# JohnLonginotto/uq

Hardware: AMD Instinct MI355X
Metric: FASTQ encode MB/s (150bp synthetic; bit-exact tables vs reference) (higher is better)
Workload: dtype u8

## Files before the change

uq_amd/csrc/pack.hip:

```cpp
#include "common.h"
#include "swar.h"
#include "lines.h"
#include "histo.h"

#ifdef PK_ROLE_CLOCK
__device__ unsigned long long pk_role_clock[16];
#define PK_CLOCK(k) do { const uint64_t now_ = __builtin_readcyclecounter(); ck_sum[(k) - 1] += now_ - ck_prev; ck_prev = now_; if ((k) == 1) ++ck_tiles; } while (0)
extern "C" int uq_pack_role_clock(unsigned long long* out16, int reset) {
    if (out16 && hipMemcpyFromSymbol(out16, HIP_SYMBOL(pk_role_clock), sizeof(pk_role_clock)) != hipSuccess) return 1;
    if (reset) {
        const unsigned long long zero[16] = {0};
        if (hipMemcpyToSymbol(HIP_SYMBOL(pk_role_clock), zero, sizeof(zero)) != hipSuccess) return 1;
    }
    return 0;
}
#else
#define PK_CLOCK(k) do { } while (0)
#endif

namespace {
constexpr int PK_THREADS = 256;

struct PackLut {
    int16_t dna_code[256];
    int16_t qual_code[256];
    int16_t n_qual[256];
};

struct PackGeom {
    uint32_t R;
    uint32_t Rs;
    uint32_t Cd, Cq;
    uint32_t G;
    uint32_t variable;
    uint32_t stage_bytes;
    uint32_t out_bytes;
    uint32_t magicG;
    uint32_t dna_max;
    uint32_t fill_d, fill_q;
    uint32_t P, magicP;
    uint32_t q_addlo, q_addhi;
    uint32_t n_char, n_code;
    uint32_t n_qchar;
    uint32_t h_shift, i2c_lo, i2c_hi, c2c_lo, c2c_hi;
};

__device__ __forceinline__ uint32_t acgt_codes(uint32_t w) { return ((w ^ (w >> 1)) >> 1) & 0x03030303u; }
__device__ __forceinline__ uint32_t acgt_chars(uint32_t codes) { return __builtin_amdgcn_perm(0u, 0x54474341u, codes); }
template <int B>
__device__ __forceinline__ uint32_t pack4(uint32_t x) {
    if (B == 8) return __builtin_amdgcn_perm(0u, x, 0x00010203u);
#ifndef PK_OLD_PACK4
    if (B <= 2) return __builtin_amdgcn_udot4(x, (1u << (3 * B)) | (1u << (2 * B + 8)) | (1u << (B + 16)) | (1u << 24), 0u, false);
    {
        const uint32_t hi = __builtin_amdgcn_udot4(x, (1u << B) | (1u << 8), 0u, false);
        return __builtin_amdgcn_udot4(x, (1u << (B + 16)) | (1u << 24), hi << (2 * B), false);
    }
#endif
    if (B == 2) return (x * 0x40100401u) >> 24;
    const uint32_t c0 = x & ((1u << B) - 1), c1 = (x >> 8) & ((1u << B) - 1), c2 = (x >> 16) & ((1u << B) - 1), c3 = x >> 24;
    return (((((c0 << B) | c1) << B) | c2) << B) | c3;
}

template <int B>
__device__ __forceinline__ uint32_t group_byte(uint32_t a0, uint32_t a1, int i) {
#ifndef PK_OLD_STORE
    if constexpr ((4 * B) % 8 == 0) return i < B / 2 ? a1 >> (8 * i) : a0 >> (8 * (i - B / 2));
    else
#endif
    return (uint32_t)((((uint64_t)a0 << (4 * B)) | a1) >> (8 * i));
}

template <bool CLEAR = false>
__device__ __noinline__ void store_tile_any(uint8_t* gdst, uint8_t* lsrc, uint32_t nb, uint32_t tid) {
    const uint32_t mis = (uint32_t)(uintptr_t)gdst;
    if ((mis & 15) == 0) {
        const uint32_t nv = nb >> 4;
        for (uint32_t i = tid; i < nv; i += 256) { ((uint4*)gdst)[i] = ((const uint4*)lsrc)[i]; if (CLEAR) ((uint4*)lsrc)[i] = make_uint4(0, 0, 0, 0); }
        for (uint32_t i = (nv << 4) + tid; i < nb; i += 256) { gdst[i] = lsrc[i]; if (CLEAR) lsrc[i] = 0; }
    } else if ((mis & 7) == 0) {
        const uint32_t nv = nb >> 3;
        for (uint32_t i = tid; i < nv; i += 256) { ((uint2*)gdst)[i] = ((const uint2*)lsrc)[i]; if (CLEAR) ((uint2*)lsrc)[i] = make_uint2(0, 0); }
        for (uint32_t i = (nv << 3) + tid; i < nb; i += 256) { gdst[i] = lsrc[i]; if (CLEAR) lsrc[i] = 0; }
    } else if ((mis & 3) == 0) {
        const uint32_t nv = nb >> 2;
        for (uint32_t i = tid; i < nv; i += 256) { ((uint32_t*)gdst)[i] = ((const uint32_t*)lsrc)[i]; if (CLEAR) ((uint32_t*)lsrc)[i] = 0; }
        for (uint32_t i = (nv << 2) + tid; i < nb; i += 256) { gdst[i] = lsrc[i]; if (CLEAR) lsrc[i] = 0; }
    } else {
        for (uint32_t i = tid; i < nb; i += 256) { gdst[i] = lsrc[i]; if (CLEAR) lsrc[i] = 0; }
    }
}
template <bool CLEAR = false>
__device__ __forceinline__ void store_tile(uint8_t* gdst, uint8_t* lsrc, uint32_t nb, uint32_t tid) {
    if ((((uint32_t)(uintptr_t)gdst) & 15u) == 0 && (nb & 15u) == 0) {
#pragma unroll 1
        for (uint32_t i = tid; i < (nb >> 4); i += 256) { ((uint4*)gdst)[i] = ((const uint4*)lsrc)[i]; if (CLEAR) ((uint4*)lsrc)[i] = make_uint4(0, 0, 0, 0); }
    } else store_tile_any<CLEAR>(gdst, lsrc, nb, tid);
}

struct alignas(16) QnLds {
    uint8_t line1[256 + 16];
    uint8_t inset[256];
    uint8_t seps[32];
    uint32_t vmin[UQ_QF_MAXC], vmax[UQ_QF_MAXC];
    uint32_t flags, on, plen, slen, nsep, l1len;
    uint32_t sepset;
    uint32_t seps_lo, seps_hi;
    uint32_t pow10[10];
};

__device__ __forceinline__ uint32_t eq_bytes(uint32_t w, uint32_t c4) {
    const uint32_t x = w ^ c4;
    return ~((((x & 0x7F7F7F7Fu) + 0x7F7F7F7Fu) | x)) & 0x80808080u;
}
__device__ __forceinline__ uint32_t nondigit_bytes(uint32_t w) {
    const uint32_t lo7 = w & 0x7F7F7F7Fu;
    return (~(lo7 + 0x50505050u) | (lo7 + 0x46464646u) | w) & 0x80808080u;
}
__device__ __forceinline__ uint32_t low_bytes(uint32_t n) { return n >= 4 ? 0xFFFFFFFFu : ~(0xFFFFFFFFu << (8 * n)); }

__device__ __forceinline__ void lds_window12(const uint8_t* base, int32_t o, uint32_t& w0, uint32_t& w1, uint32_t& w2) {
    const uint32_t* p = (const uint32_t*)(base + (o & ~3));
    const uint32_t a = p[0], b = p[1], c = p[2], d = p[3];
    const uint32_t sh = (uint32_t)o & 3u;
    w0 = __builtin_amdgcn_alignbyte(b, a, sh);
    w1 = __builtin_amdgcn_alignbyte(c, b, sh);
    w2 = __builtin_amdgcn_alignbyte(d, c, sh);
}

__device__ __forceinline__ void qname_tile(const uint8_t* stage, const uint32_t* meta, uint32_t q, QnLds* s, uint32_t* __restrict__ vals, uint64_t pitch,
                                           uint64_t row) {
    const uint32_t qs = meta[4 * q], ql = meta[4 * q + 1] - qs - 1;
    const uint32_t plen = s->plen, slen = s->slen, nsep = s->nsep, l1len = s->l1len;
    uint32_t f = 0;
    if (ql > 255) f = 2;
    else if (ql < plen + slen) f = 8;
    else {
        for (uint32_t j = 0; j < plen; j += 8) {
            uint32_t a0, a1;
            lds_window8(stage, (int32_t)(qs + j), a0, a1);
            const uint32_t l0 = *(const uint32_t*)(s->line1 + j), l1 = *(const uint32_t*)(s->line1 + j + 4);
            const uint32_t left = plen - j;
            if (((a0 ^ l0) & low_bytes(left)) | ((a1 ^ l1) & (left > 4 ? low_bytes(left - 4) : 0u))) f |= 32u;
        }
        for (uint32_t j = 0; j < slen; j += 8) {
            uint32_t a0, a1, l0, l1;
            lds_window8(stage, (int32_t)(qs + ql - slen + j), a0, a1);
            lds_window8(s->line1, (int32_t)(l1len - slen + j), l0, l1);
            const uint32_t left = slen - j;
            if (((a0 ^ l0) & low_bytes(left)) | ((a1 ^ l1) & (left > 4 ? low_bytes(left - 4) : 0u))) f |= 64u;
        }
        const uint32_t end = ql - slen;
        const uint32_t sepset = s->sepset;
        const uint32_t c0 = 0x01010101u * (sepset & 0xFFu), c1 = 0x01010101u * ((sepset >> 8) & 0xFFu), c2 = 0x01010101u * ((sepset >> 16) & 0xFFu),
                       c3 = 0x01010101u * (sepset >> 24);
        unsigned long long epos = 0, eseq = 0;
        uint32_t found = 0, differs = 0, bad = 0;
        for (uint32_t w = plen; w < ql; w += 8) {
            uint32_t a0, a1, l0, l1;
            lds_window8(stage, (int32_t)(qs + w), a0, a1);
            lds_window8(s->line1, (int32_t)w, l0, l1);
            const uint32_t inl = ql - w;
            differs |= ((a0 ^ l0) & low_bytes(inl)) | ((a1 ^ l1) & (inl > 4 ? low_bytes(inl - 4) : 0u));
            if (w >= end) continue;
            const uint32_t inm = end - w;
            const uint32_t v0 = low_bytes(inm), v1 = inm > 4 ? low_bytes(inm - 4) : 0u;
            const uint32_t sm0 = (eq_bytes(a0, c0) | eq_bytes(a0, c1) | eq_bytes(a0, c2) | eq_bytes(a0, c3)) & v0;
            const uint32_t sm1 = (eq_bytes(a1, c0) | eq_bytes(a1, c1) | eq_bytes(a1, c2) | eq_bytes(a1, c3)) & v1;
            bad |= (nondigit_bytes(a0) & ~sm0 & v0) | (nondigit_bytes(a1) & ~sm1 & v1);
            unsigned long long m = (unsigned long long)sm0 | ((unsigned long long)sm1 << 32);
            const unsigned long long bytes = (unsigned long long)a0 | ((unsigned long long)a1 << 32);
            while (m) {
                const uint32_t k = ((uint32_t)__ffsll((long long)m) - 1u) >> 3;
                m &= m - 1;
                if (found < 8) {
                    epos |= (unsigned long long)(w + k) << (8 * found);
                    eseq |= ((bytes >> (8 * k)) & 0xFFull) << (8 * found);
                }
                ++found;
            }
        }
        if (bad) f |= 16u;
        const unsigned long long want = (unsigned long long)s->seps_lo | ((unsigned long long)s->seps_hi << 32);
        if (found != nsep || eseq != want) f |= 1u;
        uint32_t start = plen;
        for (uint32_t c = 0; c <= nsep && c < UQ_QF_MAXC; ++c) {
            uint32_t stop = c == nsep ? end : (uint32_t)(epos >> (8 * c)) & 0xFFu;
            if (stop < start || stop > end) stop = start;
            const uint32_t nd = stop - start;
            uint32_t w0, w1, w2;
            lds_window12(stage, (int32_t)(qs + stop) - 12, w0, w1, w2);
            const uint32_t keep = nd > 9 ? 9u : nd;
            const uint32_t k2 = low_bytes(keep >= 4 ? 0u : 4u - keep), k1 = keep <= 4 ? 0xFFFFFFFFu : (keep >= 8 ? 0u : low_bytes(8u - keep)),
                           k0 = keep <= 8 ? 0xFFFFFFFFu : low_bytes(12u - keep);
            const uint32_t d0 = w0 & 0x0F0F0F0Fu & ~k0, d1 = w1 & 0x0F0F0F0Fu & ~k1, d2 = w2 & 0x0F0F0F0Fu & ~k2;
            uint32_t mag = d0 >> 24;
            mag = mag * 10 + (d1 & 0xFFu); mag = mag * 10 + ((d1 >> 8) & 0xFFu); mag = mag * 10 + ((d1 >> 16) & 0xFFu); mag = mag * 10 + (d1 >> 24);
            mag = mag * 10 + (d2 & 0xFFu); mag = mag * 10 + ((d2 >> 8) & 0xFFu); mag = mag * 10 + ((d2 >> 16) & 0xFFu); mag = mag * 10 + (d2 >> 24);
            if (nd > 9) f |= 4u;
            else if (nd == 0 || (nd > 1 && mag < s->pow10[nd - 1])) f |= 16u;
            vals[c * pitch + row] = mag;
            if (mag < s->vmin[c]) atomicMin(&s->vmin[c], mag);
            if (mag > s->vmax[c]) atomicMax(&s->vmax[c], mag);
            start = stop + 1;
        }
        if (ql < l1len && !differs && !(f & 32u)) f |= 128u;
        if (ql < l1len && s->line1[l1len - ql] == s->line1[0]) f |= 128u;
    }
    if (f) atomicOr(&s->flags, f);
}

constexpr int PK_NV = 5;
constexpr int PK_NV_STATS = 4;
constexpr uint32_t pk_stage_bytes(bool stats) { return (uint32_t)(stats ? PK_NV_STATS : PK_NV) * PK_THREADS * 16 + 32; }
#ifdef PK_ONE_COPY
constexpr int pks_copies(int bd, bool four_wg) { return bd == 3 ? 4 : 1; }
#else
constexpr int pks_copies(int bd, bool four_wg) { return bd == 2 && four_wg ? 8 : 4; }
#endif
constexpr uint32_t pks_bins(int bd) { return bd == 3 ? 512u : 256u; }
constexpr uint32_t pks_words(int bd, bool four_wg) { return pks_bins(bd) * pks_copies(bd, four_wg) + 128; }

struct TileRec { uint64_t start; uint32_t T, A, B, pad; };
struct PkParked { unsigned long long* bad; uq_stats* st; uq_qname_fused* qf; uint64_t first, nb, nl_total; uint32_t Rs, pad; };
struct PackLists {
    CensusView cv;
    const uint32_t* over;
};

__global__ __launch_bounds__(256) void tile_origin_kernel(CensusView cv, const unsigned long long* __restrict__ d_async, const uint32_t* __restrict__ over, uint64_t first,
                                                          uint64_t n, uint64_t R, uint64_t entries, TileRec* __restrict__ rec, unsigned long long* __restrict__ bad) {
    const uint64_t tt = (uint64_t)blockIdx.x * 256 + threadIdx.x;
    if (tt == 0) *bad = UQ_NONE;
    if (tt >= entries) return;
    uint64_t nlines = 4 * (first + n);
    if (d_async) {
        nlines = d_async[0];
        const uint64_t have = nlines / 4;
        if (have < n) n = have;
        if (d_async[1] || *over) n = 0;
    }
    uint64_t r = tt * R;
    if (r > n) r = n;
    uint32_t T, kk;
    cv_locate(cv, (int64_t)(4 * (first + r)) - 1, T, kk);
    bool ok;
    TileRec out;
    out.start = n ? cv_line_start(cv, nlines, T, kk, 0, ok) : 0;
    uint32_t c[3];
#pragma unroll
    for (uint32_t k = 0; k < 3; ++k) {
        const uint64_t t = (uint64_t)T + k;
        c[k] = t < cv.nb ? (uint32_t)((t + 1 < cv.nb ? (uint64_t)cv.offs[t + 1] : nlines) - cv.offs[t]) : 0u;
        if (c[k] > CV_LIST_CAP) c[k] = CV_LIST_CAP;
    }
    out.T = T; out.A = kk | (c[0] << 16); out.B = c[1] | (c[2] << 16); out.pad = 0;
    rec[tt] = out;
}

template <int BD, int BQ, bool NTRICK, bool FAST, bool STATS, bool QN, bool LISTS = false, bool VAR = false>
__global__ __launch_bounds__(PK_THREADS, (STATS && (NTRICK || QN)) ? 4 : 5) void pack_tile_kernel(const uint8_t* __restrict__ buf,
                                                               const uint64_t* __restrict__ ls, uint64_t first,
                                                               uint64_t n, PackLut lut, PackGeom g,
                                                               uint8_t* __restrict__ dna, uint8_t* __restrict__ qual,
                                                               unsigned long long* __restrict__ bad,
                                                               uq_stats* __restrict__ st, const unsigned long long* __restrict__ d_async,
                                                               uq_qname_fused* __restrict__ qf, uint32_t* __restrict__ qvals, uint64_t qpitch, PackLists pl,
                                                               const TileRec* __restrict__ trec) {
    constexpr int NV = STATS ? PK_NV_STATS : PK_NV;
    extern __shared__ __align__(16) uint8_t smem[];
    constexpr uint32_t STAGE_BYTES = pk_stage_bytes(STATS);
    uint8_t* stage = smem + 16;
    int16_t* l_dna = (int16_t*)(stage + STAGE_BYTES);
    int16_t* l_qual = l_dna + 256;
    int16_t* l_nq = l_qual + 256;
    QnLds* qn = (QnLds*)(l_nq + 256);
    uint32_t* meta = (uint32_t*)((uint8_t*)qn + (STATS ? sizeof(QnLds) : 0));
    uint8_t* out_d = (uint8_t*)(meta + 4 * g.R + 4);

    const uint32_t tid = threadIdx.x;
    l_dna[tid] = lut.dna_code[tid];
    l_qual[tid] = lut.qual_code[tid];
    if (NTRICK) l_nq[tid] = lut.n_qual[tid];
    RecordAcc acc;
    bool incomplete = false;
    constexpr bool FOUR_WG = STATS && (NTRICK || QN);
    constexpr int PKS_COPIES = pks_copies(BD, FOUR_WG);
    __shared__ uint32_t cnt_tab[STATS ? pks_words(BD, FOUR_WG) : 1];
    uint32_t fill_pairs = 0, n_pairs = 0;
    constexpr uint32_t PKS_BINS = pks_bins(BD), PKS_WORDS = pks_words(BD, FOUR_WG);
    if (STATS) for (uint32_t i = tid; i < PKS_WORDS; i += PK_THREADS) cnt_tab[i] = 0;
    if (VAR) for (uint32_t i = tid; i < (g.out_bytes >> 4); i += PK_THREADS) ((uint4*)out_d)[i] = make_uint4(0, 0, 0, 0);
    bool qn_on = false;
    if (STATS && QN) qn_on = qf->ok != 0;
    if (STATS && QN) {
        qn->line1[tid] = qf->line1[tid]; qn->inset[tid] = qf->inset[tid];
        if (tid < 16) qn->line1[256 + tid] = 0;
        if (tid < 32) qn->seps[tid] = qf->seps[tid];
        if (tid < UQ_QF_MAXC) { qn->vmin[tid] = 0xFFFFFFFFu; qn->vmax[tid] = 0; }
        if (tid == 0) {
            qn->flags = 0; qn->plen = qf->plen; qn->slen = qf->slen; qn->nsep = qf->nsep; qn->l1len = qf->l1len;
            uint32_t set = 0x01010101u * qf->seps[0], nset = 1, lo = 0, hi = 0;
            for (uint32_t k = 0; k < qf->nsep && k < 8; ++k) {
                const uint32_t c = qf->seps[k];
                if (k < 4) lo |= c << (8 * k); else hi |= c << (8 * (k - 4));
                bool seen = false;
                for (uint32_t m = 0; m < nset; ++m) seen = seen || ((set >> (8 * m)) & 0xFFu) == c;
                if (!seen && nset < 4) { set = (set & ~(0xFFu << (8 * nset))) | (c << (8 * nset)); ++nset; }
            }
            qn->sepset = set; qn->seps_lo = lo; qn->seps_hi = hi;
            uint32_t pw = 1;
            for (uint32_t k = 0; k < 10; ++k) { qn->pow10[k] = pw; pw *= 10; }
        }
    }
    uint32_t nr = (uint32_t)n;
#if defined(__HIP_DEVICE_COMPILE__)
    asm("" : "+s"(nr));
#endif
    uint64_t nl_total = 4 * (first + n);
    constexpr bool lists = STATS && LISTS;
    if (d_async) {
        nl_total = d_async[0];
        const uint64_t have = d_async[0] / 4;
        if (have > nr) incomplete = true; else nr = (uint32_t)have;
        if (d_async[1] || (lists && *pl.over)) { incomplete = true; nr = 0; }
    }

    __shared__ PkParked parked;
    if constexpr (FOUR_WG) {
        if (tid == 0) { parked.bad = bad; parked.st = st; parked.qf = qf; parked.first = first; parked.nb = pl.cv.nb; parked.nl_total = nl_total; parked.Rs = g.Rs; }
    }
    auto p_bad = [&] { if constexpr (FOUR_WG) return parked.bad; else return bad; };
    auto p_st = [&] { if constexpr (FOUR_WG) return parked.st; else return st; };
    auto p_qf = [&] { if constexpr (FOUR_WG) return parked.qf; else return qf; };
    auto p_first = [&] { if constexpr (FOUR_WG) return parked.first; else return first; };
    auto p_nl_total = [&] { if constexpr (FOUR_WG) return parked.nl_total; else return nl_total; };
    auto p_Rs = [&] { if constexpr (FOUR_WG) return parked.Rs; else return g.Rs; };
    auto p_cv = [&] { CensusView v = pl.cv; if constexpr (FOUR_WG) v.nb = parked.nb; return v; };
    const uint32_t R = g.R;
    const uint32_t ntiles = (nr + R - 1) / R;
    const uint32_t S = gridDim.x;
    struct Bounds { uint64_t g0, g1; uint32_t pT, pA, pB; };
    struct Regs { uint4 v[NV]; uint64_t m0; uint64_t g0; uint32_t skew, nvec, Rt, mrel, mraw; bool ok; };
    struct RawBounds { uint32_t lo, hi; };
    auto load_raw = [&](uint32_t tt) {
        RawBounds x{0u, 0u};
        if (tt < ntiles) {
            const uint32_t ln = lane_id();
            if constexpr (lists) {
                x.lo = ((const uint32_t*)(trec + tt))[ln < 8u ? ln : 0u];
            } else {
                const uint32_t Rn = (nr - tt * R) < R ? (nr - tt * R) : R;
                const uint64_t v = ls[4 * (first + (uint64_t)tt * R) + (ln == 1u ? 4 * Rn : 0u)];
                x.lo = (uint32_t)v; x.hi = (uint32_t)(v >> 32);
            }
        }
        return x;
    };
    auto bounds_of = [&](uint32_t tt, const RawBounds& x) {
        auto lane = [](uint32_t v, int k) { return (uint32_t)__builtin_amdgcn_readlane((int)v, k); };
        Bounds b{0, 0, 0, 0, 0};
        if (tt < ntiles) {
            if constexpr (lists) {
                b.g0 = (uint64_t)lane(x.lo, 0) | ((uint64_t)lane(x.lo, 1) << 32);
                b.pT = lane(x.lo, 2); b.pA = lane(x.lo, 3); b.pB = lane(x.lo, 4);
                b.g1 = (uint64_t)lane(x.lo, 6) | ((uint64_t)lane(x.lo, 7) << 32);
            } else {
                b.g0 = (uint64_t)lane(x.lo, 0) | ((uint64_t)lane(x.hi, 0) << 32);
                b.g1 = (uint64_t)lane(x.lo, 1) | ((uint64_t)lane(x.hi, 1) << 32);
            }
        }
        return b;
    };
    auto load_bounds = [&](uint32_t tt) {
        Bounds b{0, 0, 0, 0, 0};
        if (tt < ntiles) {
            const uint32_t Rn = (nr - tt * R) < R ? (nr - tt * R) : R;
            if constexpr (lists) {
                const TileRec r0 = trec[tt];
                b.g0 = r0.start; b.pT = r0.T; b.pA = r0.A; b.pB = r0.B; b.g1 = trec[tt + 1].start;
            }
            else { b.g0 = ls[4 * (first + (uint64_t)tt * R)]; b.g1 = ls[4 * (first + (uint64_t)tt * R) + 4 * Rn]; }
        }
        return b;
    };
    auto tile_reads = [&](uint32_t tt) -> uint32_t { return tt < ntiles ? ((nr - tt * R) < R ? (nr - tt * R) : R) : 0u; };
    auto issue = [&](uint32_t rfirst, uint32_t cnt, Bounds b) {
        Regs x;
        x.ok = false; x.m0 = 0; x.g0 = b.g0; x.skew = 0; x.nvec = 0; x.Rt = 0; x.mrel = 0; x.mraw = 0;
#pragma unroll
        for (int u = 0; u < NV; ++u) x.v[u] = make_uint4(0, 0, 0, 0);
        if (cnt == 0) return x;
        x.Rt = cnt;
        const uint64_t a0 = ((uint64_t)(uintptr_t)buf + b.g0) & ~uint64_t(15);
        x.skew = (uint32_t)(((uint64_t)(uintptr_t)buf + b.g0) - a0);
        const uint64_t span = b.g1 - b.g0 + x.skew;
        x.nvec = (uint32_t)((span + 15) >> 4);
        x.ok = span + 32 <= STAGE_BYTES && x.nvec <= (uint32_t)(NV * PK_THREADS);
        if constexpr (lists) {
            const uint32_t kk = b.pA & 0xFFFFu, avail = (b.pA >> 16) + (b.pB & 0xFFFFu) + (b.pB >> 16);
            if (kk + 4 * cnt > avail) x.ok = false;
        }
        if (!x.ok) return x;
        const uint4* src = (const uint4*)(buf + ((int64_t)b.g0 - (int64_t)x.skew));
#pragma unroll
        for (int u = 0; u < NV; ++u) { const uint32_t i = u * PK_THREADS + tid; if (i < x.nvec) x.v[u] = src[i]; }
        if (tid <= 4 * x.Rt) {
            if constexpr (lists) {
                uint32_t idx = (b.pA & 0xFFFFu) + tid, t = b.pT;
                const uint32_t c0 = b.pA >> 16, c1 = b.pB & 0xFFFFu;
                if (idx > c0) { idx -= c0; ++t; if (idx > c1) { idx -= c1; ++t; } }
                x.mrel = x.skew - (uint32_t)b.g0 + (idx == 0 ? 0u : (uint32_t)t * (uint32_t)CV_TILE - pl.cv.mis + 1u);
                x.mraw = idx == 0 ? 0u : (uint32_t)pl.cv.list[(uint64_t)t * CV_LIST_CAP + (idx - 1)];
            } else x.m0 = ls[4 * (first + (uint64_t)rfirst) + tid];
        }
        return x;
    };

    uint32_t rr, pp;
    fast_divmod(tid, g.P, g.magicP, rr, pp);
    uint32_t badr = 0xFFFFFFFFu;
    uint32_t bad_tile = 0xFFFFFFFFu;
#ifdef PK_ROLE_CLOCK
    uint64_t ck_prev = 0, ck_sum[5] = {0, 0, 0, 0, 0};
    uint32_t ck_tiles = 0;
#endif
    auto do_tile = [&](const uint32_t r0, const Regs& cur, auto&& between) {
        const uint32_t Rt = cur.Rt;
        uint8_t* out_q = out_d + ((Rt * g.Cd + 15) & ~15u);
        if (cur.ok) {
            if (tid <= 4 * Rt) meta[tid] = lists ? cur.mrel + cur.mraw : (uint32_t)(cur.m0 - cur.g0) + cur.skew;
#pragma unroll
            for (int u = 0; u < NV; ++u) { const uint32_t i = u * PK_THREADS + tid; if (i < cur.nvec) ((uint4*)stage)[i] = cur.v[u]; }
        } else {
            if (tid == 0) bad_tile = bad_tile < r0 ? bad_tile : r0;
            incomplete = true;
            if (STATS && QN && qn_on && tid == 0) atomicOr(&p_qf()->flags, 256u);
        }
        __syncthreads();
        const bool ok = cur.ok;
        PK_CLOCK(1);
#ifndef PK_QN_NO_PRIO
        if (STATS && QN && tid >= PK_THREADS - 64) __builtin_amdgcn_s_setprio(3);
#endif
        between();
#ifndef PK_ABL_NOQN
        if (STATS && QN && qn_on && ok && tid >= PK_THREADS - 64 && tid - (PK_THREADS - 64) < Rt)
            qname_tile(stage, meta, tid - (PK_THREADS - 64), qn, qvals, qpitch, (uint64_t)r0 + (tid - (PK_THREADS - 64)));
#endif
#ifndef PK_QN_NO_PRIO
        if (STATS && QN && tid >= PK_THREADS - 64) __builtin_amdgcn_s_setprio(0);
#endif
        if (ok) {
            auto pack_group = [&](const uint32_t r, const uint32_t L, const int32_t wd, const uint32_t shd, const int32_t wq, const uint32_t shq, uint8_t* orow_d,
                                  uint8_t* orow_q, const uint32_t gg) {
                const int32_t j0 = (int32_t)L - 8 * (int32_t)gg - 8;
                uint32_t ad0 = 0, ad1 = 0, aq0 = 0, aq1 = 0;
                if (j0 > -8) {
                uint32_t b_lo, b_hi, q_lo, q_hi;
                lds_window8_at(stage, wd, shd, b_lo, b_hi);
                lds_window8_at(stage, wq, shq, q_lo, q_hi);
                if (j0 < 0) {
                    uint32_t mlo, mhi;
                    window_masks((uint32_t)(-j0), mlo, mhi);
                    b_lo = bfi(mlo, b_lo, g.fill_d); b_hi = bfi(mhi, b_hi, g.fill_d);
                    q_lo = bfi(mlo, q_lo, g.fill_q); q_hi = bfi(mhi, q_hi, g.fill_q);
                }
                bool generic = !FAST;
                if (FAST) {
                    uint32_t c0, c1, e0, e1;
                    if constexpr (BD == 2) {
                        c0 = acgt_codes(b_lo); c1 = acgt_codes(b_hi);
                        e0 = acgt_chars(c0) ^ b_lo; e1 = acgt_chars(c1) ^ b_hi;
                    } else {
                        c0 = __builtin_amdgcn_perm(g.i2c_hi, g.i2c_lo, (b_lo >> g.h_shift) & 0x07070707u);
                        c1 = __builtin_amdgcn_perm(g.i2c_hi, g.i2c_lo, (b_hi >> g.h_shift) & 0x07070707u);
                        e0 = __builtin_amdgcn_perm(g.c2c_hi, g.c2c_lo, c0) ^ b_lo; e1 = __builtin_amdgcn_perm(g.c2c_hi, g.c2c_lo, c1) ^ b_hi;
                    }
                    uint32_t u0 = q_lo + g.q_addlo, u1 = q_hi + g.q_addlo;
                    uint32_t bq0 = (q_lo | (q_lo + g.q_addhi) | ~u0) & 0x80808080u;
                    uint32_t bq1 = (q_hi | (q_hi + g.q_addhi) | ~u1) & 0x80808080u;
                    uint32_t x0 = u0 & 0x7F7F7F7Fu, x1 = u1 & 0x7F7F7F7Fu;
                    if (e0 | e1) {
                        if (NTRICK && !((q_lo | q_hi) & 0x80808080u)) {
                            const uint32_t m0 = nonzero_bytes(e0), m1 = nonzero_bytes(e1);
                            if (((b_lo ^ g.n_char) & m0) | ((b_hi ^ g.n_char) & m1)) generic = true;
                            c0 &= ~m0; c1 &= ~m1;
                            x0 = bfi(m0, g.n_code, x0); x1 = bfi(m1, g.n_code, x1);
                            bq0 &= ~m0; bq1 &= ~m1;
                        } else generic = true;
                    }
                    if (bq0 | bq1) generic = true;
                    ad0 = pack4<BD>(c0); ad1 = pack4<BD>(c1);
                    aq0 = pack4<BQ>(x0); aq1 = pack4<BQ>(x1);
                    if (STATS) {
                        if (generic) incomplete = true;
#ifdef PK_ABL_NOCOUNT
                        else if (false) {
#else
                        else {
#endif
                            uint8_t* hb = (uint8_t*)cnt_tab + ((lane_id() & (PKS_COPIES - 1)) << 2);
                            if constexpr (BD == 2) {
                                const uint32_t bin0 = (c0 << 6) | x0, bin1 = (c1 << 6) | x1;
#pragma unroll
                                for (int k = 0; k < 4; ++k) {
                                    if constexpr (PKS_COPIES == 1) {
                                        atomicAdd(&cnt_tab[(bin0 >> (8 * k)) & 0xFFu], 1u);
                                        atomicAdd(&cnt_tab[(bin1 >> (8 * k)) & 0xFFu], 1u);
                                    } else {
                                        atomicAdd((uint32_t*)(hb + (((bin0 >> (8 * k)) & 0xFFu) * (4 * PKS_COPIES))), 1u);
                                        atomicAdd((uint32_t*)(hb + (((bin1 >> (8 * k)) & 0xFFu) * (4 * PKS_COPIES))), 1u);
                                    }
                                }
                            } else {
#pragma unroll
                                for (int k = 0; k < 4; ++k) {
                                    const uint32_t b0 = (((c0 >> (8 * k)) & 7u) << 6) | ((x0 >> (8 * k)) & 63u), b1 = (((c1 >> (8 * k)) & 7u) << 6) | ((x1 >> (8 * k)) & 63u);
                                    atomicAdd((uint32_t*)(hb + b0 * (4 * PKS_COPIES)), 1u);
                                    atomicAdd((uint32_t*)(hb + b1 * (4 * PKS_COPIES)), 1u);
                                }
                            }
                            if (j0 < 0) fill_pairs += (uint32_t)(-j0);
                            if (NTRICK && (e0 | e1)) {
                                const uint32_t m0 = nonzero_bytes(e0), m1 = nonzero_bytes(e1);
                                const uint32_t ne0 = nonzero_bytes(q_lo ^ g.n_qchar), ne1 = nonzero_bytes(q_hi ^ g.n_qchar);
                                n_pairs += (uint32_t)__popc(m0 & 0x01010101u) + (uint32_t)__popc(m1 & 0x01010101u);
                                if ((m0 & ne0) | (m1 & ne1)) incomplete = true;
                            }
                        }
                    }
                }
                if (generic) {
                    const uint32_t cbw[2] = {b_lo, b_hi};
                    const uint32_t cqw[2] = {q_lo, q_hi};
                    uint32_t ad[2] = {0, 0}, aq[2] = {0, 0};
                    int32_t orall = 0;
#pragma unroll
                    for (int k = 0; k < 8; ++k) {
                        const uint32_t cb = (cbw[k >> 2] >> (8 * (k & 3))) & 255u;
                        const uint32_t cc = (cqw[k >> 2] >> (8 * (k & 3))) & 255u;
                        int32_t dc = l_dna[cb];
                        int32_t qc = l_qual[cc];
                        if (NTRICK) {
                            if (dc < 0) { dc = 0; qc = l_nq[cb]; }
                        }
                        orall |= dc | qc;
                        ad[k >> 2] = (ad[k >> 2] << BD) | (uint32_t)dc;
                        aq[k >> 2] = (aq[k >> 2] << BQ) | (uint32_t)qc;
                    }
                    if (orall < 0) {
                        badr = badr < r0 + r ? badr : r0 + r;
                        ad[0] = ad[1] = aq[0] = aq[1] = 0;
                    }
                    ad0 = ad[0]; ad1 = ad[1]; aq0 = aq[0]; aq1 = aq[1];
                }
                }
                if (g.variable) {
                    const int32_t i = (int32_t)L - 8 * (int32_t)gg;
                    if (i >= 0 && i < 4) { ad1 |= 1u << (BD * i); aq1 |= 1u << (BQ * i); }
                    else if (i >= 4 && i < 8) { ad0 |= 1u << (BD * (i - 4)); aq0 |= 1u << (BQ * (i - 4)); }
                }
                uint8_t* od = orow_d - BD * gg;
                uint8_t* oq = orow_q - BQ * gg;
#ifdef PK_ABL_NOSTORE
                if ((ad0 ^ aq0) == 0x12345678u && (ad1 ^ aq1) == 0x9ABCDEF0u) od[0] = 1;
                else if (false)
#endif
                if (gg + 1 < g.G) {
#pragma unroll
                    for (int i = 0; i < BD; ++i) od[-i] = (uint8_t)group_byte<BD>(ad0, ad1, i);
#pragma unroll
                    for (int i = 0; i < BQ; ++i) oq[-i] = (uint8_t)group_byte<BQ>(aq0, aq1, i);
                } else {
                    const uint32_t nd = g.Cd - BD * gg, nq = g.Cq - BQ * gg;
#pragma unroll
                    for (int i = 0; i < BD; ++i)
                        if ((uint32_t)i < nd) od[-i] = (uint8_t)group_byte<BD>(ad0, ad1, i);
#pragma unroll
                    for (int i = 0; i < BQ; ++i)
                        if ((uint32_t)i < nq) oq[-i] = (uint8_t)group_byte<BQ>(aq0, aq1, i);
                }
            };
            if (rr < Rt) {
                const uint32_t r = rr;
                const uint32_t so = meta[4 * r + 1];
                uint32_t L = meta[4 * r + 2] - so - 1;
                const uint32_t qo = meta[4 * r + 3];
                if (STATS) {
                    const uint32_t Lq = meta[4 * r + 4] - qo - 1;
#ifndef PK_ABL_NOREC
                    if (pp == 0) acc.record(r0 + r, stage[meta[4 * r + 2]] == '+', L, Lq, meta[4 * r + 4] - meta[4 * r]);
#endif
                    if (L > g.dna_max || Lq != L) incomplete = true;
                }
                if (L > g.dna_max || meta[4 * r + 4] - qo - 1 != L) { badr = badr < r0 + r ? badr : r0 + r; L = 0; }
                uint8_t* orow_d = out_d + r * g.Cd + (g.Cd - 1);
                uint8_t* orow_q = out_q + r * g.Cq + (g.Cq - 1);
                const uint32_t gend = VAR ? (((L + 8) >> 3) < g.G ? ((L + 8) >> 3) : g.G) : g.G;
#ifndef PK_ABL_NOGROUP
                int32_t wd = (int32_t)(so + L) - 8 * (int32_t)pp - 8, wq = (int32_t)(qo + L) - 8 * (int32_t)pp - 8;
                const uint32_t shd = (uint32_t)wd & 3u, shq = (uint32_t)wq & 3u;
                wd &= ~3; wq &= ~3;
                const int32_t wstep = 8 * (int32_t)g.P;
                for (uint32_t gg = pp; gg < gend; gg += g.P, wd -= wstep, wq -= wstep) pack_group(r, L, wd, shd, wq, shq, orow_d, orow_q, gg);
#endif
            }
        }
        PK_CLOCK(2);
        __syncthreads();
        PK_CLOCK(3);
#ifndef PK_NO_EARLY_WAIT
        __builtin_amdgcn_s_waitcnt(0x0F70);
#endif
        PK_CLOCK(4);
        if (ok) {
            if constexpr (STATS && (NTRICK || QN)) {
                store_tile<VAR>(dna + (uint64_t)r0 * g.Cd, out_d, Rt * g.Cd, tid);
                store_tile<VAR>(qual + (uint64_t)r0 * g.Cq, out_q, Rt * g.Cq, tid);
            } else {
                store_tile_any<VAR>(dna + (uint64_t)r0 * g.Cd, out_d, Rt * g.Cd, tid);
                store_tile_any<VAR>(qual + (uint64_t)r0 * g.Cq, out_q, Rt * g.Cq, tid);
            }
        }
        PK_CLOCK(5);
    };

    uint32_t t = blockIdx.x;
    constexpr bool VBOUNDS = STATS && (NTRICK || QN);
    using NextBounds = std::conditional_t<VBOUNDS, RawBounds, Bounds>;
    auto fetch_next = [&](uint32_t tt) -> NextBounds { if constexpr (VBOUNDS) return load_raw(tt); else return load_bounds(tt); };
    auto next_bounds = [&](uint32_t tt, const NextBounds& x) -> Bounds { if constexpr (VBOUNDS) return bounds_of(tt, x); else return x; };
    NextBounds b_next = fetch_next(t + S);
    Regs cur = issue(t * R, tile_reads(t), load_bounds(t));
#ifndef PK_NO_EARLY_WAIT
    __builtin_amdgcn_s_waitcnt(0x0F70);
#endif
#ifdef PK_ROLE_CLOCK
    ck_prev = __builtin_readcyclecounter();
#endif
    for (; t < ntiles; t += S) {
        NextBounds b_nn{};
        if constexpr (!VBOUNDS) b_nn = fetch_next(t + 2 * S);
        if (cur.ok) {
            const Regs now = cur;
            do_tile(t * R, now, [&] {
                cur = issue((t + S) * R, tile_reads(t + S), next_bounds(t + S, b_next));
                if constexpr (VBOUNDS) b_next = fetch_next(t + 2 * S); else b_next = b_nn;
            });
        } else {
            const uint32_t Rt = cur.Rt;
            __syncthreads();
            const uint32_t Rs = p_Rs();
            for (uint32_t sub = 0; sub < Rt; sub += Rs) {
                const uint32_t cnt = Rt - sub < Rs ? Rt - sub : Rs;
                const uint32_t rf = t * R + sub;
                Bounds sb{0, 0, 0, 0, 0};
                if constexpr (lists) {
                    uint32_t T, kk; bool found;
                    const CensusView cv = p_cv();
                    const uint64_t nl_total = p_nl_total();
                    cv_locate(cv, (int64_t)(4 * (p_first() + rf)) - 1, T, kk);
                    sb.g0 = cv_line_start(cv, nl_total, T, kk, 0, found); sb.g1 = cv_line_start(cv, nl_total, T, kk, 4 * cnt, found);
                    uint32_t c[3];
#pragma unroll
                    for (uint32_t k = 0; k < 3; ++k) {
                        const uint64_t tq = (uint64_t)T + k;
                        c[k] = tq < cv.nb ? (uint32_t)((tq + 1 < cv.nb ? (uint64_t)cv.offs[tq + 1] : nl_total) - cv.offs[tq]) : 0u;
                        if (c[k] > CV_LIST_CAP) c[k] = CV_LIST_CAP;
                    }
                    sb.pT = T; sb.pA = kk | (c[0] << 16); sb.pB = c[1] | (c[2] << 16);
                } else { sb.g0 = ls[4 * (first + (uint64_t)rf)]; sb.g1 = ls[4 * (first + (uint64_t)rf) + 4 * cnt]; }
                const Regs piece = issue(rf, cnt, sb);
                do_tile(rf, piece, [] {});
                __syncthreads();
            }
            cur = issue((t + S) * R, tile_reads(t + S), next_bounds(t + S, b_next));
            if constexpr (VBOUNDS) b_next = fetch_next(t + 2 * S); else b_next = b_nn;
#ifndef PK_NO_EARLY_WAIT
            __builtin_amdgcn_s_waitcnt(0x0F70);
#endif
        }
    }
#ifdef PK_ROLE_CLOCK
    if (lane_id() == 0) {
        unsigned long long* ck = pk_role_clock + (STATS && QN && tid >= PK_THREADS - 64 ? 8 : 0);
        for (int k = 0; k < 5; ++k) atomicAdd(ck + k, (unsigned long long)ck_sum[k]);
        atomicAdd(ck + 5, (unsigned long long)ck_tiles); atomicAdd(ck + 6, 1ull);
    }
#endif
    if (badr != 0xFFFFFFFFu) atomicMin(p_bad(), (unsigned long long)badr);
    if (bad_tile != 0xFFFFFFFFu) atomicMin(p_bad(), (unsigned long long)bad_tile);
    if (STATS) {
        if (fill_pairs) atomicSub(&cnt_tab[lane_id() & (PKS_COPIES - 1)], fill_pairs);
        if (NTRICK && n_pairs) {
            atomicSub(&cnt_tab[((g.n_code & 0xFFu) * PKS_COPIES) + (lane_id() & (PKS_COPIES - 1))], n_pairs);
            atomicAdd(&cnt_tab[PKS_BINS * PKS_COPIES], n_pairs);
        }
        __syncthreads();
        const uint32_t qmin = 0x80u - (g.q_addlo & 0xFFu);
        uq_stats* const st = p_st();
        uq_qname_fused* const qf = p_qf();
        for (uint32_t bin = tid; bin < PKS_BINS; bin += PK_THREADS) {
            uint32_t v = 0;
#pragma unroll
            for (int c = 0; c < PKS_COPIES; ++c) v += cnt_tab[bin * PKS_COPIES + c];
            const uint32_t code = bin >> 6;
            const uint32_t base = BD == 2 ? (0x54474341u >> (8 * code)) & 0xFFu
                                          : ((code < 4 ? g.c2c_lo >> (8 * code) : g.c2c_hi >> (8 * (code - 4))) & 0xFFu);
            if (v) atomicAdd((unsigned long long*)&st->counts[base * 256 + qmin + (bin & 63u)], (unsigned long long)v);
        }
        if (NTRICK && tid == 0) {
            const uint32_t v = cnt_tab[PKS_BINS * PKS_COPIES];
            if (v) atomicAdd((unsigned long long*)&st->counts[(g.n_char & 0xFFu) * 256 + (g.n_qchar & 0xFFu)], (unsigned long long)v);
        }
        acc.flush(st, p_first());
        if (incomplete) st->reserved = 1;
        if (QN) {
            if (qn_on && tid < UQ_QF_MAXC && qn->vmin[tid] <= qn->vmax[tid]) { atomicMin(&qf->vmin[tid], qn->vmin[tid]); atomicMax(&qf->vmax[tid], qn->vmax[tid]); }
            if (qn_on && tid == 0 && qn->flags) atomicOr(&qf->flags, qn->flags);
            if (blockIdx.x == 0 && tid == 0) qf->nreads = nr;
        }
    }
}

__global__ __launch_bounds__(256) void pack_carry_kernel(const uint8_t* __restrict__ buf, const uint64_t* __restrict__ ls,
                                                         uint64_t first, uint64_t n, PackLut lut, uint32_t bd, uint32_t bq,
                                                         uint32_t Cd, uint32_t Cq, uint32_t variable,
                                                         uint8_t* __restrict__ dna, uint8_t* __restrict__ qual,
                                                         unsigned long long* __restrict__ bad) {
    __shared__ int16_t l_dna[256], l_qual[256], l_nq[256];
    l_dna[threadIdx.x] = lut.dna_code[threadIdx.x];
    l_qual[threadIdx.x] = lut.qual_code[threadIdx.x];
    l_nq[threadIdx.x] = lut.n_qual[threadIdx.x];
    __syncthreads();
    const uint64_t r = (uint64_t)blockIdx.x * blockDim.x + threadIdx.x;
    if (r >= n) return;
    const uint64_t* p = ls + 4 * (first + r);
    const uint64_t s = p[1], q = p[3];
    const uint32_t L = (uint32_t)(p[2] - s - 1);
    uint8_t* drow = dna + r * Cd;
    uint8_t* qrow = qual + r * Cq;
    uint32_t td = 0, tq = 0, bdn = 0, bqn = 0;
    int32_t pd = (int32_t)Cd - 1, pq = (int32_t)Cq - 1;
    for (uint32_t t = 0; t < L; ++t) {
        uint32_t cb = buf[s + L - 1 - t], cc = buf[q + L - 1 - t];
        int dc = l_dna[cb], qc = l_qual[cc];
        if (dc < 0) { dc = 0; qc = l_nq[cb]; }
        if (qc < 0) { atomicMin(bad, (unsigned long long)r); qc = 0; }
        td += (uint32_t)dc << bdn; tq += (uint32_t)qc << bqn;
        bdn += bd; bqn += bq;
        while (bdn > 8) { bdn -= 8; if (pd >= 0) drow[pd] = (uint8_t)td; td >>= 8; --pd; }
        while (bqn > 8) { bqn -= 8; if (pq >= 0) qrow[pq] = (uint8_t)tq; tq >>= 8; --pq; }
    }
    td += variable << bdn; tq += variable << bqn;
    while (pd >= 0) { drow[pd] = (uint8_t)td; td >>= 8; --pd; }
    while (pq >= 0) { qrow[pq] = (uint8_t)tq; tq >>= 8; --pq; }
}

typedef void (*PackKernel)(const uint8_t*, const uint64_t*, uint64_t, uint64_t, PackLut, PackGeom, uint8_t*, uint8_t*, unsigned long long*,
                           uq_stats*, const unsigned long long*, uq_qname_fused*, uint32_t*, uint64_t, PackLists, const TileRec*);

template <int BD, int BQ>
PackKernel pick_nt(bool ntrick, bool fast) {
    if ((BD == 2 || BD == 3) && fast) return ntrick ? pack_tile_kernel<(BD == 3 ? 3 : 2), BQ, true, true, false, false> : pack_tile_kernel<(BD == 3 ? 3 : 2), BQ, false, true, false, false>;
    return ntrick ? pack_tile_kernel<BD, BQ, true, false, false, false> : pack_tile_kernel<BD, BQ, false, false, false, false>;
}

template <int BD, bool QN, bool LISTS = false, bool VAR = false>
PackKernel pick_stats_kernel_q(int bq, bool ntrick) {
#define UQ_PS(B) case B: return ntrick ? pack_tile_kernel<BD, B, true, true, true, QN, LISTS, VAR> : pack_tile_kernel<BD, B, false, true, true, QN, LISTS, VAR>;
    switch (bq) { UQ_PS(1) UQ_PS(2) UQ_PS(3) UQ_PS(4) UQ_PS(5) default: return ntrick ? pack_tile_kernel<BD, 6, true, true, true, QN, LISTS, VAR> : pack_tile_kernel<BD, 6, false, true, true, QN, LISTS, VAR>; }
#undef UQ_PS
}
PackKernel pick_stats_kernel(int bd, int bq, bool ntrick, bool qn, bool lists, bool var) {
    if (var && lists) {
        if (qn) return bd == 3 ? pick_stats_kernel_q<3, true, true, true>(bq, ntrick) : pick_stats_kernel_q<2, true, true, true>(bq, ntrick);
        return bd == 3 ? pick_stats_kernel_q<3, false, true, true>(bq, ntrick) : pick_stats_kernel_q<2, false, true, true>(bq, ntrick);
    }
    if (qn && lists) return bd == 3 ? pick_stats_kernel_q<3, true, true>(bq, ntrick) : pick_stats_kernel_q<2, true, true>(bq, ntrick);
    if (lists) return bd == 3 ? pick_stats_kernel_q<3, false, true>(bq, ntrick) : pick_stats_kernel_q<2, false, true>(bq, ntrick);
    if (bd == 3) return qn ? pick_stats_kernel_q<3, true>(bq, ntrick) : pick_stats_kernel_q<3, false>(bq, ntrick);
    return qn ? pick_stats_kernel_q<2, true>(bq, ntrick) : pick_stats_kernel_q<2, false>(bq, ntrick);
}

template <int BD>
PackKernel pick_bq(int bq, bool ntrick, bool fast) {
    switch (bq) {
        case 1: return pick_nt<BD, 1>(ntrick, fast); case 2: return pick_nt<BD, 2>(ntrick, fast); case 3: return pick_nt<BD, 3>(ntrick, fast);
        case 4: return pick_nt<BD, 4>(ntrick, fast); case 5: return pick_nt<BD, 5>(ntrick, fast); case 6: return pick_nt<BD, 6>(ntrick, fast);
        case 7: return pick_nt<BD, 7>(ntrick, fast); default: return pick_nt<BD, 8>(ntrick, fast);
    }
}

PackKernel pick_kernel(int bd, int bq, bool ntrick, bool fast) {
    switch (bd) {
        case 1: return pick_bq<1>(bq, ntrick, fast); case 2: return pick_bq<2>(bq, ntrick, fast); case 3: return pick_bq<3>(bq, ntrick, fast);
        case 4: return pick_bq<4>(bq, ntrick, fast); case 5: return pick_bq<5>(bq, ntrick, fast); case 6: return pick_bq<6>(bq, ntrick, fast);
        case 7: return pick_bq<7>(bq, ntrick, fast); default: return pick_bq<8>(bq, ntrick, fast);
    }
}
}

static int pack_impl(uq_ctx* ctx, const uint8_t* d_buf, const uint64_t* d_line_start, uint64_t first_read,
                     uint64_t nreads, const uq_pack_params* hp, uint8_t* d_dna, uint8_t* d_qual, uint64_t* d_bad,
                     uq_stats* d_stats, int* h_fused, const unsigned long long* d_async = nullptr, uq_qname_fused* d_q = nullptr,
                     uint32_t* d_vals = nullptr, uint64_t vals_pitch = 0) {
    const bool use_lists = d_line_start == nullptr && d_async != nullptr && d_stats != nullptr;
    UQ_REQUIRE(nreads <= (1ull << 31), "uq_pack: %llu reads in one call (at most 2^31)", (unsigned long long)nreads);
    UQ_REQUIRE(ctx && d_buf && (d_line_start || use_lists) && hp && d_dna && d_qual && d_bad, "uq_pack: null argument");
    UQ_REQUIRE(!use_lists || (ctx->async_buf == d_buf && ctx->async_nbytes > 0), "uq_pack_stats_async: no line index given and no census of this buffer queued in front");
    if (h_fused) *h_fused = 0;
    ctx->pk_stats = ctx->pk_q = nullptr;
    if (d_stats && ctx->stats_sent == (const void*)d_stats) ctx->stats_sent = nullptr;
    UQ_REQUIRE(hp->bits_per_base >= 1 && hp->bits_per_base <= 8 && hp->bits_per_quality >= 1 && hp->bits_per_quality <= 8,
               "uq_pack: bits per symbol must be 1..8");
    const uint32_t bd = hp->bits_per_base, bq = hp->bits_per_quality;
    const uint32_t Cd = hp->dna_bytes_per_row, Cq = hp->quality_bytes_per_row;
    const uint32_t Lv = hp->dna_max + (hp->variable ? 1 : 0);
    UQ_REQUIRE(Cd == (bd * Lv + 7) / 8 && Cq == (bq * Lv + 7) / 8,
               "uq_pack: row bytes (%u, %u) do not match ceil(bits * (dna_max + variable) / 8)", Cd, Cq);
    struct BadGuard {
        uint64_t* p; hipStream_t s; bool armed;
        ~BadGuard() { if (armed) (void)hipMemsetAsync(p, 0xFF, 8, s); }
    } bad_guard{d_bad, ctx->stream, use_lists && nreads != 0};
    if (!bad_guard.armed) UQ_CHECK_HIP(hipMemsetAsync(d_bad, 0xFF, 8, ctx->stream));
    if (nreads == 0) return 0;

    PackLut lut;
    int max_d = 0, max_q = 0;
    bool ntrick = false;
    int fill_d = -1, fill_q = -1;
    for (int i = 0; i < 256; ++i) {
        lut.dna_code[i] = hp->dna_code[i];
        lut.qual_code[i] = hp->qual_code[i];
        lut.n_qual[i] = (int16_t)(hp->n_qual[i] > 32767 ? 32767 : hp->n_qual[i]);
        if (hp->dna_code[i] > max_d) max_d = hp->dna_code[i];
        if (hp->qual_code[i] > max_q) max_q = hp->qual_code[i];
        if (hp->dna_code[i] < 0 && hp->n_qual[i] >= 0) { ntrick = true; if (hp->n_qual[i] > max_q) max_q = hp->n_qual[i]; }
        if (hp->dna_code[i] == 0 && fill_d < 0) fill_d = i;
        if (hp->qual_code[i] == 0 && fill_q < 0) fill_q = i;
    }
    UQ_REQUIRE(fill_d >= 0 && fill_q >= 0, "uq_pack: the alphabets need a symbol with code 0");
    UQ_REQUIRE(max_d < (1 << bd), "uq_pack: a DNA code does not fit %u bits", bd);
    const bool carry = max_q >= (1 << bq);
    const uint32_t stage_cap = (d_stats ? PK_NV_STATS : PK_NV) * PK_THREADS * 16;
    const uint32_t rec = (uint32_t)hp->max_record_bytes;
    UQ_REQUIRE(rec >= 4, "uq_pack: max_record_bytes not set (take it from uq_stats)");

    if (carry || rec + 64 > stage_cap) {
        if (d_stats) return 0;
        uint32_t blocks = (uint32_t)((nreads + 255) / 256);
        pack_carry_kernel<<<blocks, 256, 0, ctx->stream>>>(d_buf, d_line_start, first_read, nreads, lut, bd, bq, Cd, Cq,
                                                           hp->variable ? 1u : 0u, d_dna, d_qual, (unsigned long long*)d_bad);
        UQ_LAUNCH_CHECK();
        return 0;
    }

    PackGeom g;
    g.Cd = Cd; g.Cq = Cq; g.variable = hp->variable ? 1 : 0;
    g.G = (Lv + 7) / 8;
    g.dna_max = (uint32_t)hp->dna_max;
    g.magicG = magic_u32(g.G);
    g.fill_d = 0x01010101u * (uint32_t)fill_d;
    g.fill_q = 0x01010101u * (uint32_t)fill_q;
    uint32_t Rs = (stage_cap - 64) / rec;
    if (Rs > (PK_THREADS - 1) / 4) Rs = (PK_THREADS - 1) / 4;
    if (Rs == 0) Rs = 1;
    uint32_t R = Rs;
    const uint32_t avg = (uint32_t)hp->avg_record_bytes;
    if (avg >= 4 && avg < rec) {
        R = (stage_cap - 64) / (avg + avg * 15 / 100 + 1);
        if (R > (PK_THREADS - 1) / 4) R = (PK_THREADS - 1) / 4;
        if (R < Rs) R = Rs;
    }
    {
        const uint32_t out_cap = stage_cap * 3 / 4, fit = out_cap / (Cd + Cq);
        if (R > fit) R = fit > Rs ? fit : Rs;
    }
    if (R >= 4) {
        const uint32_t r16 = R & ~15u, r8 = R & ~7u, r4 = R & ~3u;
        if (r16 * 100 >= R * 85) R = r16; else if (r8 * 100 >= R * 85) R = r8; else R = r4;
    }
    if (R == 0) R = 1;
    if (Rs > R) Rs = R;
    g.R = R; g.Rs = Rs;
    g.stage_bytes = pk_stage_bytes(d_stats != nullptr);
    g.out_bytes = (((R * Cd + 15) & ~15u) + R * Cq + 15) & ~15u;
    uint32_t P = (d_q ? PK_THREADS - 64 : PK_THREADS) / R;
    if (P > g.G) P = g.G;
    if (P < 1) P = 1;
    g.P = P; g.magicP = magic_u32(P);
    bool fast = bd == 2 && hp->dna_code['A'] == 0 && hp->dna_code['C'] == 1 && hp->dna_code['G'] == 2 && hp->dna_code['T'] == 3;
    int nbases = 0, nq = 0, qmin = 256, qmaxc = -1, ntrick_bases = 0, nchar = 0;
    for (int i = 0; i < 256; ++i) {
        if (hp->dna_code[i] >= 0) ++nbases;
        if (hp->qual_code[i] >= 0) { ++nq; if (i < qmin) qmin = i; if (i > qmaxc) qmaxc = i; }
        if (hp->dna_code[i] < 0 && hp->n_qual[i] >= 0) { ++ntrick_bases; nchar = i; }
    }
    g.h_shift = g.i2c_lo = g.i2c_hi = g.c2c_lo = g.c2c_hi = 0;
    bool fast3 = false;
    if (bd == 3 && nbases >= 1 && nbases <= 8) {
        for (uint32_t sh = 0; sh <= 4 && !fast3; ++sh) {
            uint8_t i2c[8], c2c[8]; bool used[8] = {false, false, false, false, false, false, false, false};
            memset(i2c, 0, 8); memset(c2c, 0, 8);
            bool ok = true;
            for (int ch = 1; ch < 128 && ok; ++ch) {
                const int code = hp->dna_code[ch];
// ... 118 lines not shown
```

Before: 1.530 million.

## Add straight-line fast path for full interior groups before generic pack loop

Adds a specialized loop over fully populated 8-symbol groups. It drops the tail masking and the fill/variable-length handling, and uses wave-wide ballots to bail out to the generic pack_group path on any error or non-fast symbol. The histogram atomics move into a shared count_pairs lambda. Byte stores to LDS now go through a volatile address-space-3 pointer, likely to stop the compiler merging or reordering them. This trades extra code size and a wave-uniform early break for fewer branches per group in the common case.

```diff
diff --git a/uq_amd/csrc/pack.hip b/uq_amd/csrc/pack.hip
--- a/uq_amd/csrc/pack.hip
+++ b/uq_amd/csrc/pack.hip
@@ -69,6 +69,13 @@
     else
 #endif
     return (uint32_t)((((uint64_t)a0 << (4 * B)) | a1) >> (8 * i));
+}
+__device__ __forceinline__ void lds_store8(uint8_t* p, uint32_t v) {
+#ifdef PK_MERGED_STORES
+    *p = (uint8_t)v;
+#else
+    *(volatile __attribute__((address_space(3))) uint8_t*)p = (uint8_t)v;
+#endif
 }
 
 template <bool CLEAR = false>
@@ -452,6 +459,29 @@
         if (STATS && QN && tid >= PK_THREADS - 64) __builtin_amdgcn_s_setprio(0);
 #endif
         if (ok) {
+            auto count_pairs =[&](const uint32_t c0, const uint32_t c1, const uint32_t x0, const uint32_t x1) {
+                uint8_t* hb = (uint8_t*)cnt_tab + ((lane_id() & (PKS_COPIES - 1)) << 2);
+                if constexpr (BD == 2) {
+                    const uint32_t bin0 = (c0 << 6) | x0, bin1 = (c1 << 6) | x1;
+#pragma unroll
+                    for (int k = 0; k < 4; ++k) {
+                        if constexpr (PKS_COPIES == 1) {
+                            atomicAdd(&cnt_tab[(bin0 >> (8 * k)) & 0xFFu], 1u);
+                            atomicAdd(&cnt_tab[(bin1 >> (8 * k)) & 0xFFu], 1u);
+                        } else {
+                            atomicAdd((uint32_t*)(hb + (((bin0 >> (8 * k)) & 0xFFu) * (4 * PKS_COPIES))), 1u);
+                            atomicAdd((uint32_t*)(hb + (((bin1 >> (8 * k)) & 0xFFu) * (4 * PKS_COPIES))), 1u);
+                        }
+                    }
+                } else {
+#pragma unroll
+                    for (int k = 0; k < 4; ++k) {
+                        const uint32_t b0 = (((c0 >> (8 * k)) & 7u) << 6) | ((x0 >> (8 * k)) & 63u), b1 = (((c1 >> (8 * k)) & 7u) << 6) | ((x1 >> (8 * k)) & 63u);
+                        atomicAdd((uint32_t*)(hb + b0 * (4 * PKS_COPIES)), 1u);
+                        atomicAdd((uint32_t*)(hb + b1 * (4 * PKS_COPIES)), 1u);
+                    }
+                }
+            };
             auto pack_group = [&](const uint32_t r, const uint32_t L, const int32_t wd, const uint32_t shd, const int32_t wq, const uint32_t shq, uint8_t* orow_d,
                                   uint8_t* orow_q, const uint32_t gg) {
                 const int32_t j0 = (int32_t)L - 8 * (int32_t)gg - 8;
@@ -500,27 +530,7 @@
 #else
                         else {
 #endif
-                            uint8_t* hb = (uint8_t*)cnt_tab + ((lane_id() & (PKS_COPIES - 1)) << 2);
-                            if constexpr (BD == 2) {
-                                const uint32_t bin0 = (c0 << 6) | x0, bin1 = (c1 << 6) | x1;
-#pragma unroll
-                                for (int k = 0; k < 4; ++k) {
-                                    if constexpr (PKS_COPIES == 1) {
-                                        atomicAdd(&cnt_tab[(bin0 >> (8 * k)) & 0xFFu], 1u);
-                                        atomicAdd(&cnt_tab[(bin1 >> (8 * k)) & 0xFFu], 1u);
-                                    } else {
-                                        atomicAdd((uint32_t*)(hb + (((bin0 >> (8 * k)) & 0xFFu) * (4 * PKS_COPIES))), 1u);
-                                        atomicAdd((uint32_t*)(hb + (((bin1 >> (8 * k)) & 0xFFu) * (4 * PKS_COPIES))), 1u);
-                                    }
-                                }
-                            } else {
-#pragma unroll
-                                for (int k = 0; k < 4; ++k) {
-                                    const uint32_t b0 = (((c0 >> (8 * k)) & 7u) << 6) | ((x0 >> (8 * k)) & 63u), b1 = (((c1 >> (8 * k)) & 7u) << 6) | ((x1 >> (8 * k)) & 63u);
-                                    atomicAdd((uint32_t*)(hb + b0 * (4 * PKS_COPIES)), 1u);
-                                    atomicAdd((uint32_t*)(hb + b1 * (4 * PKS_COPIES)), 1u);
-                                }
-                            }
+                            count_pairs(c0, c1, x0, x1);
                             if (j0 < 0) fill_pairs += (uint32_t)(-j0);
                             if (NTRICK && (e0 | e1)) {
                                 const uint32_t m0 = nonzero_bytes(e0), m1 = nonzero_bytes(e1);
@@ -569,17 +579,17 @@
 #endif
                 if (gg + 1 < g.G) {
 #pragma unroll
-                    for (int i = 0; i < BD; ++i) od[-i] = (uint8_t)group_byte<BD>(ad0, ad1, i);
-#pragma unroll
-                    for (int i = 0; i < BQ; ++i) oq[-i] = (uint8_t)group_byte<BQ>(aq0, aq1, i);
+                    for (int i = 0; i < BD; ++i) lds_store8(od - i, group_byte<BD>(ad0, ad1, i));
+#pragma unroll
+                    for (int i = 0; i < BQ; ++i) lds_store8(oq - i, group_byte<BQ>(aq0, aq1, i));
                 } else {
                     const uint32_t nd = g.Cd - BD * gg, nq = g.Cq - BQ * gg;
 #pragma unroll
                     for (int i = 0; i < BD; ++i)
-                        if ((uint32_t)i < nd) od[-i] = (uint8_t)group_byte<BD>(ad0, ad1, i);
+                        if ((uint32_t)i < nd) lds_store8(od - i, group_byte<BD>(ad0, ad1, i));
 #pragma unroll
                     for (int i = 0; i < BQ; ++i)
-                        if ((uint32_t)i < nq) oq[-i] = (uint8_t)group_byte<BQ>(aq0, aq1, i);
+                        if ((uint32_t)i < nq) lds_store8(oq - i, group_byte<BQ>(aq0, aq1, i));
                 }
             };
             if (rr < Rt) {
@@ -603,7 +613,61 @@
                 const uint32_t shd = (uint32_t)wd & 3u, shq = (uint32_t)wq & 3u;
                 wd &= ~3; wq &= ~3;
                 const int32_t wstep = 8 * (int32_t)g.P;
-                for (uint32_t gg = pp; gg < gend; gg += g.P, wd -= wstep, wq -= wstep) pack_group(r, L, wd, shd, wq, shq, orow_d, orow_q, gg);
+                uint32_t gg = pp;
+#if !defined(PK_NO_STRAIGHT) && !defined(PK_ABL_NOSTORE)
+                if constexpr (FAST) {
+                    const uint32_t gfull = L >> 3;
+                    for (; gg < gfull; gg += g.P, wd -= wstep, wq -= wstep) {
+                        uint32_t b_lo, b_hi, q_lo, q_hi;
+                        lds_window8_at(stage, wd, shd, b_lo, b_hi);
+                        lds_window8_at(stage, wq, shq, q_lo, q_hi);
+                        uint32_t c0, c1, e0, e1;
+                        if constexpr (BD == 2) {
+                            c0 = acgt_codes(b_lo); c1 = acgt_codes(b_hi);
+                            e0 = acgt_chars(c0) ^ b_lo; e1 = acgt_chars(c1) ^ b_hi;
+                        } else {
+                            c0 = __builtin_amdgcn_perm(g.i2c_hi, g.i2c_lo, (b_lo >> g.h_shift) & 0x07070707u);
+                            c1 = __builtin_amdgcn_perm(g.i2c_hi, g.i2c_lo, (b_hi >> g.h_shift) & 0x07070707u);
+                            e0 = __builtin_amdgcn_perm(g.c2c_hi, g.c2c_lo, c0) ^ b_lo; e1 = __builtin_amdgcn_perm(g.c2c_hi, g.c2c_lo, c1) ^ b_hi;
+                        }
+                        const uint32_t u0 = q_lo + g.q_addlo, u1 = q_hi + g.q_addlo;
+                        uint32_t bq0 = (q_lo | (q_lo + g.q_addhi) | ~u0) & 0x80808080u, bq1 = (q_hi | (q_hi + g.q_addhi) | ~u1) & 0x80808080u;
+                        uint32_t x0 = u0 & 0x7F7F7F7Fu, x1 = u1 & 0x7F7F7F7Fu;
+                        uint32_t err = e0 | e1, n_here = 0, n_other_q = 0;
+                        if constexpr (NTRICK) {
+                            if (__builtin_amdgcn_ballot_w64(err != 0)) {
+                                const uint32_t m0 = nonzero_bytes(e0), m1 = nonzero_bytes(e1);
+                                err = ((b_lo ^ g.n_char) & m0) | ((b_hi ^ g.n_char) & m1) | ((q_lo | q_hi) & 0x80808080u);
+                                c0 &= ~m0; c1 &= ~m1;
+                                x0 = bfi(m0, g.n_code, x0); x1 = bfi(m1, g.n_code, x1);
+                                bq0 &= ~m0; bq1 &= ~m1;
+                                if constexpr (STATS) {
+                                    n_here = (uint32_t)__popc(m0 & 0x01010101u) + (uint32_t)__popc(m1 & 0x01010101u);
+                                    n_other_q = (m0 & nonzero_bytes(q_lo ^ g.n_qchar)) | (m1 & nonzero_bytes(q_hi ^ g.n_qchar));
+                                }
+                            }
+                        }
+                        if (__builtin_amdgcn_ballot_w64((err | bq0 | bq1) != 0)) break;
+                        const uint32_t ad0 = pack4<BD>(c0), ad1 = pack4<BD>(c1), aq0 = pack4<BQ>(x0), aq1 = pack4<BQ>(x1);
+                        if constexpr (STATS) {
+#ifndef PK_ABL_NOCOUNT
+                            count_pairs(c0, c1, x0, x1);
+#endif
+                            if constexpr (NTRICK) {
+                                n_pairs += n_here;
+                                if (n_other_q) incomplete = true;
+                            }
+                        }
+                        uint8_t* od = orow_d - BD * gg;
+                        uint8_t* oq = orow_q - BQ * gg;
+#pragma unroll
+                        for (int i = 0; i < BD; ++i) lds_store8(od - i, group_byte<BD>(ad0, ad1, i));
+#pragma unroll
+                        for (int i = 0; i < BQ; ++i) lds_store8(oq - i, group_byte<BQ>(aq0, aq1, i));
+                    }
+                }
+#endif
+                for (; gg < gend; gg += g.P, wd -= wstep, wq -= wstep) pack_group(r, L, wd, shd, wq, shq, orow_d, orow_q, gg);
 #endif
             }
         }
```

Result: faster. 1.640 million, median of 6 (+7.2%).
